# YaoZengzeng/yustack

Measured on AMD Instinct MI355X. Metric: GiB/s device-resident Internet checksum, batched packets, 1/2/4/8 MI355X, higher is better.
Workload: dtype u32; 1 GPU; config3: 1M x 1500-B TCP segments incl. pseudo-header (sendTCP field value); packets_per_gpu=1048576, packet_bytes=1500, mode=tcp, rotating_batches=2, kernel=k_small<16,6>, parallelism=shard1 (independent packets, no collective; one rank per GPU), backend=none

## Files before the change

### yustack_amd/csrc/yucsum_kernels.hip

```cpp
#include <hip/hip_runtime.h>

#include <stdint.h>

#include <atomic>
#include <type_traits>

#include "yucsum.h"
#include "yucsum_internal.h"
#include "yucsum_plan.h"

namespace {

constexpr uint32_t kSelSwap = 0x02030001u;
constexpr uint32_t kSelIdent = 0x03020100u;
using yu::kLEMax;

struct BatchArgs {
  const uint8_t *data;
  const uint64_t *offsets;
  const uint16_t *initial_arr;
  const uint8_t *addrs;
  uint16_t *out;
  uint8_t *fill;
  uint64_t stride;
  uint64_t n;
  uint64_t end;
  uint32_t len;
  uint32_t initial;
  uint32_t uf;
  uint32_t xcd;
  uint32_t small_waves;
  int mode;
};

__host__ __device__ __forceinline__ bool mode_is_ipv4(int m) {
  return m == YU_MODE_IPV4 || m == YU_MODE_VERIFY_IPV4;
}
using yu::l4_field;
using yu::l4_min;
using yu::mode_field;
using yu::mode_fills;
using yu::mode_is_tx;
__host__ __device__ __forceinline__ bool mode_has_pseudo(int m) {
  return m == YU_MODE_UDP || m == YU_MODE_TCP || m == YU_MODE_VERIFY_TCP ||
         m == YU_MODE_VERIFY_UDP;
}
__host__ __device__ __forceinline__ uint32_t mode_proto(int m) {
  return (m == YU_MODE_TCP || m == YU_MODE_VERIFY_TCP) ? 6u : 17u;
}
__host__ __device__ __forceinline__ uint32_t min_len(int m) {
  switch (m) {
    case YU_MODE_UDP: return 8;
    case YU_MODE_TCP: return 20;
    case YU_MODE_ICMP: return 4;
    case YU_MODE_IPV4:
    case YU_MODE_VERIFY_IPV4: return 1;
    default: return 0;
  }
}

__device__ __forceinline__ uint32_t fold32(uint32_t v) {
  uint32_t w = (v & 0xFFFFu) + (v >> 16);
  return (w + (w >> 16)) & 0xFFFFu;
}

__device__ __forceinline__ uint32_t sad(uint32_t x, uint32_t acc) {
  return __builtin_amdgcn_sad_u16(x, 0u, acc);
}

__device__ __forceinline__ uint32_t sadperm(uint32_t x, uint32_t sel,
                                            uint32_t acc) {
  return __builtin_amdgcn_sad_u16(__builtin_amdgcn_perm(x, x, sel), 0u, acc);
}

template <bool BE>
__device__ __forceinline__ uint32_t add_word(uint32_t x, uint32_t sel,
                                             uint32_t acc) {
  return BE ? sadperm(x, sel, acc) : sad(x, acc);
}

__device__ __forceinline__ uint32_t le_to_be(uint32_t s_le, uint32_t odd) {
  const uint32_t r = fold32(s_le);
  return odd ? r : (((r & 0xFFu) << 8) | (r >> 8));
}

template <int G>
__device__ __forceinline__ uint32_t group_total(uint32_t v) {
  static_assert(G >= 1 && G <= 64 && (G & (G - 1)) == 0, "G must be a power of two");
  if (G >= 2) v += (uint32_t)__builtin_amdgcn_update_dpp(0, (int)v, 0x111, 0xf, 0xf, true);
  if (G >= 4) v += (uint32_t)__builtin_amdgcn_update_dpp(0, (int)v, 0x112, 0xf, 0xf, true);
  if (G >= 8) v += (uint32_t)__builtin_amdgcn_update_dpp(0, (int)v, 0x114, 0xf, 0xf, true);
  if (G >= 16) v += (uint32_t)__builtin_amdgcn_update_dpp(0, (int)v, 0x118, 0xf, 0xf, true);
  if (G >= 32) v += (uint32_t)__builtin_amdgcn_update_dpp(0, (int)v, 0x142, 0xa, 0xf, false);
  if (G >= 64) v += (uint32_t)__builtin_amdgcn_update_dpp(0, (int)v, 0x143, 0xc, 0xf, false);
  return v;
}

__device__ __forceinline__ uint32_t wave_or(uint32_t v) {
  v |= (uint32_t)__builtin_amdgcn_update_dpp(0, (int)v, 0x111, 0xf, 0xf, true);
  v |= (uint32_t)__builtin_amdgcn_update_dpp(0, (int)v, 0x112, 0xf, 0xf, true);
  v |= (uint32_t)__builtin_amdgcn_update_dpp(0, (int)v, 0x114, 0xf, 0xf, true);
  v |= (uint32_t)__builtin_amdgcn_update_dpp(0, (int)v, 0x118, 0xf, 0xf, true);
  v |= (uint32_t)__builtin_amdgcn_update_dpp(0, (int)v, 0x142, 0xa, 0xf, false);
  v |= (uint32_t)__builtin_amdgcn_update_dpp(0, (int)v, 0x143, 0xc, 0xf, false);
  return (uint32_t)__shfl((int)v, 63, 64);
}

__device__ __forceinline__ uint64_t grid_wave(uint32_t xcd) {
  const uint32_t b = blockIdx.x, n = gridDim.x;
  uint32_t lb = b;
  if (xcd) {
    const uint32_t x = b & 7u, i = b >> 3, q = n >> 3, r = n & 7u;
    lb = (x < r ? x * (q + 1u) : r * (q + 1u) + (x - r) * q) + i;
  }
  return (uint64_t)lb * (blockDim.x >> 6) +
         (uint64_t)__builtin_amdgcn_readfirstlane(threadIdx.x >> 6);
}

typedef unsigned int u32x4 __attribute__((ext_vector_type(4)));

__device__ __forceinline__ uint64_t uniform64(uint64_t x) {
  const uint32_t lo = __builtin_amdgcn_readfirstlane((uint32_t)x);
  const uint32_t hi = __builtin_amdgcn_readfirstlane((uint32_t)(x >> 32));
  return ((uint64_t)hi << 32) | lo;
}

__device__ __forceinline__ uint64_t readlane64(uint64_t v, uint32_t l) {
  return ((uint64_t)(uint32_t)__builtin_amdgcn_readlane((int)(uint32_t)(v >> 32), l) << 32) |
         (uint32_t)__builtin_amdgcn_readlane((int)(uint32_t)v, l);
}

__device__ __forceinline__ uint64_t shfl64(uint64_t v, uint32_t src) {
  const uint32_t lo = (uint32_t)__shfl((int)(uint32_t)v, (int)src, 64);
  const uint32_t hi = (uint32_t)__shfl((int)(uint32_t)(v >> 32), (int)src, 64);
  return ((uint64_t)hi << 32) | lo;
}

using yu::kOOB;

__device__ __forceinline__ __amdgpu_buffer_rsrc_t rsrc_at(uint64_t base,
                                                          uint64_t end) {
  end = (end + 3u) & ~3ull;
  const uint64_t n = end > base ? end - base : 0;
  return __builtin_amdgcn_make_buffer_rsrc((void *)base, (short)0,
                                           (int)(n < kOOB ? n : kOOB), 0x00020000);
}

__device__ __forceinline__ uint4 bld16(__amdgpu_buffer_rsrc_t r, uint32_t off,
                                       bool nt) {
  const u32x4 t = nt ? __builtin_amdgcn_raw_buffer_load_b128(r, (int)off, 0, 2)
                     : __builtin_amdgcn_raw_buffer_load_b128(r, (int)off, 0, 0);
  return make_uint4(t.x, t.y, t.z, t.w);
}

template <int NT>
__device__ __forceinline__ constexpr bool nt_step(int u, int U) {
  return NT == 1 || (NT == 2 && u != 0 && u != U - 1);
}

struct Junk {
  uint32_t off[3];
  uint32_t mask[3];
};

__device__ __forceinline__ Junk make_junk(uint32_t sh, uint32_t E, int mode) {
  Junk j;
  j.off[0] = 0u;
  j.mask[0] = (1u << (8u * sh)) - 1u;
  const uint32_t f = mode_field(mode);
  const bool fld = mode_is_tx(mode) && sh + f + 2u <= E;
  const uint32_t fr = sh + f;
  const uint32_t fb = fr & 3u;
  j.off[1] = fr & ~3u;
  j.mask[1] = !fld ? 0u : (fb == 3u ? 0xFF000000u : (0xFFFFu << (8u * fb)));
  j.off[2] = (fr & ~3u) + 4u;
  j.mask[2] = (fld && fb == 3u) ? 0xFFu : 0u;
  return j;
}

__device__ __forceinline__ uint32_t pick_dword(const uint4 &c, uint32_t q) {
  return q == 0 ? c.x : (q == 1 ? c.y : (q == 2 ? c.z : c.w));
}

template <int LG>
__device__ __forceinline__ void junk_take(const uint4 &c0, uint32_t gbase,
                                          const Junk &j, uint32_t (&x)[3]) {
  static_assert(LG >= 1, "junk chunks 0/1 must sit in different lanes of step 0");
#pragma unroll
  for (int k = 0; k < 3; ++k) {
    const uint32_t d = j.off[k];
    x[k] = __shfl(pick_dword(c0, (d >> 2) & 3u), (int)(gbase + (d >> 4)), 64);
  }
}

template <bool BE>
__device__ __forceinline__ uint32_t junk_sum(const uint32_t (&x)[3],
                                             const Junk &j, uint32_t sel) {
  uint32_t s = 0;
#pragma unroll
  for (int k = 0; k < 3; ++k) s = add_word<BE>(x[k] & j.mask[k], sel, s);
  return s;
}

__device__ uint32_t g_side_zero[2] = {0u, 0u};

struct Side {
  uint32_t a, b;
  uint16_t i;
};

struct SidePtrs {
  const uint8_t *a;
  const uint8_t *i;
  uint32_t as, is;
};

__device__ __forceinline__ SidePtrs side_ptrs(const BatchArgs &A) {
  SidePtrs s;
  const bool use_addrs = A.addrs && mode_has_pseudo(A.mode);
  s.a = use_addrs ? A.addrs : (const uint8_t *)g_side_zero;
  s.as = use_addrs ? 8u : 0u;
  s.i = A.initial_arr ? (const uint8_t *)A.initial_arr : (const uint8_t *)g_side_zero;
  s.is = A.initial_arr ? 2u : 0u;
  return s;
}

__device__ __forceinline__ Side load_side(const SidePtrs &sp, uint64_t p) {
  const uint32_t *a = (const uint32_t *)(sp.a + p * sp.as);
  Side s;
  s.a = a[0];
  s.b = a[1];
  s.i = *(const uint16_t *)(sp.i + p * sp.is);
  return s;
}

__device__ __forceinline__ uint32_t packet_value(const BatchArgs &A, uint32_t v, uint64_t len,
                                                 const Side &sd) {
  const int mode = A.mode;
  if (mode == YU_MODE_RAW) {
    v += A.initial_arr ? sd.i : A.initial;
  } else if (mode_has_pseudo(mode)) {
    uint32_t ph;
    if (A.addrs) {
      ph = sadperm(sd.a, kSelSwap, 0u);
      ph = sadperm(sd.b, kSelSwap, ph);
      ph += mode_proto(mode);
    } else {
      ph = A.initial_arr ? sd.i : A.initial;
    }
    v += ph + (uint32_t)(len & 0xFFFFu);
  }
  uint32_t r = fold32(v);
  if (mode_is_tx(mode)) r = (~r) & 0xFFFFu;
  return r;
}

__device__ __forceinline__ void store_field(const BatchArgs &A, uint32_t r, uint8_t *pkt,
                                            uint32_t hdr_end) {
  const int mode = A.mode;
  if (A.fill && pkt && mode_is_tx(mode)) {
    const uint32_t f = mode_field(mode);
    if (f + 2u <= hdr_end) {
      uint8_t *q = pkt + f;
      const uint16_t be = (uint16_t)((r >> 8) | (r << 8));
      if (((uintptr_t)q & 1u) == 0 && !A.offsets) {
        __builtin_nontemporal_store(be, (uint16_t *)q);
      } else if (((uintptr_t)q & 1u) == 0) {
        *(uint16_t *)q = be;
      } else {
        q[0] = (uint8_t)(r >> 8);
        q[1] = (uint8_t)r;
      }
    }
  }
}

struct Extent {
  uint64_t hi;
};
__device__ __forceinline__ Extent batch_extent(const BatchArgs &A) {
  Extent e;
  e.hi = A.offsets ? A.offsets[A.n] : ~0ull;
  return e;
}

__device__ __forceinline__ uint8_t *fill_at(const BatchArgs &A, const Extent &x, uint64_t off,
                                            uint64_t len) {
  const bool in = len <= YU_MAX_TRANSPORT_LEN && off <= x.hi && len <= x.hi - off;
  return A.fill && in ? A.fill + off : nullptr;
}

__device__ __forceinline__ void finish_packet(const BatchArgs &A, uint64_t p,
                                              uint32_t v, uint64_t len,
                                              const Side &sd, uint8_t *pkt,
                                              uint32_t hdr_end) {
  const uint32_t r = packet_value(A, v, len, sd);
  if (A.out) A.out[p] = (uint16_t)r;
  store_field(A, r, pkt, hdr_end);
}

__device__ __forceinline__ uint32_t tail_cut(uint32_t x, int cr, int lim,
                                             uint32_t tm) {
  return cr < lim ? x : (cr == lim ? (x & tm) : 0u);
}

template <bool BE>
__device__ __forceinline__ uint32_t sum_masked(const uint4 &c, int cr,
                                               const int (&lim)[4], uint32_t tm,
                                               uint32_t sel, uint32_t acc) {
  acc = add_word<BE>(tail_cut(c.x, cr, lim[0], tm), sel, acc);
  acc = add_word<BE>(tail_cut(c.y, cr, lim[1], tm), sel, acc);
  acc = add_word<BE>(tail_cut(c.z, cr, lim[2], tm), sel, acc);
  acc = add_word<BE>(tail_cut(c.w, cr, lim[3], tm), sel, acc);
  return acc;
}

template <bool BE>
__device__ __forceinline__ uint32_t sum_full(const uint4 &c, uint32_t sel,
                                             uint32_t acc) {
  acc = add_word<BE>(c.x, sel, acc);
  acc = add_word<BE>(c.y, sel, acc);
  acc = add_word<BE>(c.z, sel, acc);
  acc = add_word<BE>(c.w, sel, acc);
  return acc;
}

__device__ __forceinline__ uint32_t ipv4_hl(uint32_t w0, uint32_t sh) {
  return ((w0 >> (8u * sh)) & 0xFu) * 4u;
}

template <int G, int U>
struct SmallItem {
  uint4 c[U];
  Side sd;
  uint32_t sh, len;
};

template <int G, int U, int NT, bool SIDE = true>
__device__ __forceinline__ void small_fetch(const BatchArgs &A,
                                            const SidePtrs &sp, uint64_t pb,
                                            uint32_t gw, uint32_t gl, bool ipv4,
                                            SmallItem<G, U> &it) {
  const uint64_t p = pb + gw;
  const bool active = p < A.n;
  const uint64_t data = (uint64_t)(uintptr_t)A.data;
  const uint64_t base = uniform64((data + pb * A.stride) & ~3ull);
  const uint64_t sabs = data + (active ? p : pb) * A.stride;
  const uint32_t lw = (uint32_t)((sabs & ~3ull) - base);
  it.sh = (uint32_t)(sabs & 3u);
  it.len = active ? A.len : 0u;
  const uint32_t le = ipv4 ? (it.len < 60u ? it.len : 60u) : it.len;
  const uint32_t eload = active ? it.sh + le : 0u;
  const __amdgpu_buffer_rsrc_t r = rsrc_at(base, A.end);
#pragma unroll
  for (int u = 0; u < U; ++u) {
    const uint32_t cr = 16u * (gl + (uint32_t)u * G);
    it.c[u] = bld16(r, cr < eload ? lw + cr : kOOB, nt_step<NT>(u, U));
  }
  if (SIDE) it.sd = load_side(sp, active ? p : A.n - 1);
}

template <int G, int U, int NT, int PR = 0>
__global__ __launch_bounds__(256) void k_small(BatchArgs A) {
  constexpr int GPW = 64 / G;
  constexpr int SPR = PR ? PR / GPW : 1;
  static_assert(PR == 0 || (PR % GPW == 0 && PR <= 64 && (SPR & (SPR - 1)) == 0),
                "a run is whole wave steps and fits the wave's lanes");
  const uint32_t lane = threadIdx.x & 63u;
  const uint32_t gl = lane & (G - 1);
  const uint32_t gw = lane / G;
  const uint64_t wave = grid_wave(A.xcd);
  const uint64_t nwaves = (uint64_t)gridDim.x * (blockDim.x >> 6);
  const int mode = A.mode;
  const bool ipv4 = mode_is_ipv4(mode);
  const SidePtrs sp = side_ptrs(A);
  const uint32_t uf = A.uf;
  auto first = [&](uint64_t t) -> uint64_t {
    if (PR == 0) return (wave + t * nwaves) * GPW;
    return (wave + t / SPR * nwaves) * PR + (t % SPR) * GPW;
  };

  uint64_t t = 0;
  uint64_t pb = first(0);
  if (pb >= A.n) return;
  uint32_t res = 0;
  Side rs, nrs;
  constexpr bool kDppSide = G <= 16;
  auto run_side = [&](uint64_t q, Side &d) __attribute__((always_inline)) {
    uint64_t x = q + lane;
    bool own = lane < (uint32_t)PR;
    if (kDppSide) {
      const uint32_t jj = (uint32_t)(G - 1) - gl;
      x = q + (uint64_t)jj * GPW + gw;
      own = jj < (uint32_t)SPR;
    }
    d = load_side(sp, own && x < A.n ? x : (q < A.n ? q : A.n - 1));
  };
  auto step = [&](const SmallItem<G, U> &it, SmallItem<G, U> &nx) __attribute__((always_inline)) -> bool {
    const uint64_t pn = first(t + 1);
    const bool more = pn < A.n;
    const uint32_t k = (uint32_t)(t % SPR);
    small_fetch<G, U, NT, PR == 0>(A, sp, more ? pn : A.n, gw, gl, ipv4, nx);
    if (PR && k == 0 && t) rs = nrs;
    if (PR && k == SPR - 1 && more) run_side(pn, nrs);

    uint32_t E = it.sh + it.len;
    if (ipv4) {
      const uint32_t hl = __shfl(ipv4_hl(it.c[0].x, it.sh), (int)(lane & ~(uint32_t)(G - 1)), 64);
      E = it.sh + (it.len < hl ? it.len : hl);
    }
    const int F = (int)(E & ~3u);
    const int lim[4] = {F, F - 4, F - 8, F - 12};
    const uint32_t tm = (1u << (8u * (E & 3u))) - 1u;
    uint32_t acc = 0;
#pragma unroll
    for (int u = 0; u < U; ++u) {
      const int cr = 16 * (int)(gl + (uint32_t)u * G);
      if ((uint32_t)u < uf)
        acc = sum_full<false>(it.c[u], 0u, acc);
      else
        acc = sum_masked<false>(it.c[u], cr, lim, tm, 0u, acc);
    }
    const uint64_t p = pb + gw;
    const Junk j = make_junk(it.sh, E, mode);
    uint32_t jx[3] = {0u, 0u, 0u};
    if (PR && kDppSide) {
      uint32_t own = 0;
#pragma unroll
      for (int i = 0; i < 3; ++i)
        if ((j.off[i] >> 4) == gl) own = sad(pick_dword(it.c[0], (j.off[i] >> 2) & 3u) & j.mask[i], own);
      acc -= own;
    } else {
      junk_take<__builtin_ctz(G)>(it.c[0], lane & ~(uint32_t)(G - 1), j, jx);
    }
    acc = group_total<G>(acc);
    if (PR == 0) {
      if (gl == G - 1 && p < A.n) {
        const uint32_t v = le_to_be(acc - junk_sum<false>(jx, j, 0u), it.sh & 1u);
        finish_packet(A, p, v, it.len, it.sd,
                      A.fill ? A.fill + p * A.stride : nullptr, E - it.sh);
      }
    } else {
      Side sd;
      if (kDppSide) {
        sd = rs;
        rs.a = (uint32_t)__builtin_amdgcn_update_dpp(0, (int)rs.a, 0x111, 0xf, 0xf, true);
        rs.b = (uint32_t)__builtin_amdgcn_update_dpp(0, (int)rs.b, 0x111, 0xf, 0xf, true);
        rs.i = (uint16_t)__builtin_amdgcn_update_dpp(0, (int)(uint32_t)rs.i, 0x111, 0xf, 0xf, true);
      } else {
        const int src = (int)(k * GPW + gw);
        sd.a = (uint32_t)__shfl((int)rs.a, src, 64);
        sd.b = (uint32_t)__shfl((int)rs.b, src, 64);
        sd.i = (uint16_t)__shfl((int)rs.i, src, 64);
      }
      const uint32_t v = le_to_be(acc - (kDppSide ? 0u : junk_sum<false>(jx, j, 0u)), it.sh & 1u);
      const uint32_t r = packet_value(A, v, it.len, sd);
      if (gl == G - 1 && p < A.n && A.fill) store_field(A, r, A.fill + p * A.stride, E - it.sh);
      const uint32_t got = (uint32_t)__shfl((int)r, (int)((lane % GPW) * G + G - 1), 64);
      res = lane / GPW == k ? got : res;
      if (k == SPR - 1 || !more) {
        const uint64_t q = pb - (uint64_t)k * GPW + lane;
        if (lane < (uint32_t)PR && q < A.n && A.out) A.out[q] = (uint16_t)res;
      }
    }
    pb = pn;
    ++t;
    return more;
  };
  SmallItem<G, U> a, b;
  small_fetch<G, U, NT, PR == 0>(A, sp, pb, gw, gl, ipv4, a);
  if (PR) run_side(pb, rs);
  for (;;) {
    if (!step(a, b)) break;
    if (!step(b, a)) break;
  }
}

template <int G>
struct TinyItem {
  uint4 c[G];
  Side sd;
};

template <int G, int NT>
__device__ __forceinline__ void tiny_fetch(const BatchArgs &A, const SidePtrs &sp,
                                           uint64_t pb, uint32_t g, uint32_t j,
                                           TinyItem<G> &it) {
  constexpr uint32_t GPW = 64 / G;
  const uint64_t base = uniform64((uint64_t)(uintptr_t)A.data + pb * A.stride);
  const __amdgpu_buffer_rsrc_t r = rsrc_at(base, A.end);
  const bool in = 16u * j < A.len;
#pragma unroll
  for (int k = 0; k < G; ++k) {
    const uint32_t q = GPW * (uint32_t)k + g;
    const bool active = in && pb + q < A.n;
    it.c[k] = bld16(r, active ? (uint32_t)(q * A.stride) + 16u * j : kOOB, NT != 0);
  }
  const uint64_t pf = pb + GPW * j + g;
  it.sd = load_side(sp, pf < A.n ? pf : A.n - 1);
}

template <int G>
__device__ __forceinline__ uint32_t bcast_last(uint32_t v, uint32_t lane) {
  if (G == 4)
    return (uint32_t)__builtin_amdgcn_update_dpp(0, (int)v, 0xFF, 0xf, 0xf, false);
  return (uint32_t)__shfl(v, (int)(lane | (G - 1)), 64);
}

template <int G>
__device__ __forceinline__ void tiny_store(const BatchArgs &A, uint64_t pb, uint32_t g, uint32_t j,
                                           const TinyItem<G> &it, uint32_t be, uint32_t f) {
  constexpr uint32_t GPW = 64 / G;
  const uint64_t e4 = A.end & ~3ull;
  const uint32_t fd = (f >> 2) & 3u, sh = (f & 2u) * 8u;
  const uint32_t m = 0xFFFFu << sh;
  const bool holder = j == (f >> 4);
  const bool in = 16u * j < A.len;
#pragma unroll
  for (int k = 0; k < G; ++k) {
    const uint32_t v = ((uint32_t)__shfl((int)be, (int)(g * G + (uint32_t)k), 64)) << sh;
    uint4 c = it.c[k];
    if (holder) {
      c.x = fd == 0 ? (c.x & ~m) | v : c.x;
      c.y = fd == 1 ? (c.y & ~m) | v : c.y;
      c.z = fd == 2 ? (c.z & ~m) | v : c.z;
      c.w = fd == 3 ? (c.w & ~m) | v : c.w;
    }
    const uint64_t q = pb + GPW * (uint32_t)k + g;
    uint32_t *dst = (uint32_t *)(A.fill + q * A.stride + 16u * j);
    const uint64_t da = (uint64_t)(uintptr_t)dst;
    if (in && q < A.n) {
      if (da + 16u <= e4) {
        *(uint4 *)dst = c;
      } else {
        if (da + 4u <= e4) dst[0] = c.x;
        if (da + 8u <= e4) dst[1] = c.y;
        if (da + 12u <= e4) dst[2] = c.z;
      }
    }
  }
}

template <int G, int NT, bool WB = false>
__global__ __launch_bounds__(256) void k_tiny(BatchArgs A) {
  constexpr uint32_t GPW = 64 / G;
  const uint32_t lane = threadIdx.x & 63u;
  const uint32_t j = lane & (G - 1);
  const uint32_t g = lane / G;
  const uint64_t wave = grid_wave(A.xcd);
  const uint64_t step = (uint64_t)gridDim.x * (blockDim.x >> 6) * 64u;
  const SidePtrs sp = side_ptrs(A);
  const uint32_t E = A.len;
  const int F = (int)(E & ~3u);
  const int lim[4] = {F, F - 4, F - 8, F - 12};
  const uint32_t tm = (1u << (8u * (E & 3u))) - 1u;
  const bool full = A.uf != 0;
  const uint32_t f = mode_field(A.mode);
  const uint32_t fm = (mode_is_tx(A.mode) && j == f / 16u) ? ~(0xFFFFu << (8u * (f & 3u))) : ~0u;
  const uint32_t fd = (f >> 2) & 3u;
  const uint4 m4 = make_uint4(fd == 0 ? fm : ~0u, fd == 1 ? fm : ~0u, fd == 2 ? fm : ~0u,
                              fd == 3 ? fm : ~0u);
  const bool wb = WB && A.fill && A.stride >= ((A.len + 15u) & ~15u);

  uint64_t pb = wave * 64u;
  if (pb >= A.n) return;
  TinyItem<G> it;
  tiny_fetch<G, NT>(A, sp, pb, g, j, it);
  for (;;) {
    const uint64_t pn = pb + step;
    const bool more = pn < A.n;
    TinyItem<G> nx;
    tiny_fetch<G, NT>(A, sp, more ? pn : A.n, g, j, nx);

    uint32_t mine = 0;
#pragma unroll
    for (int k = 0; k < G; ++k) {
      const uint4 c = make_uint4(it.c[k].x & m4.x, it.c[k].y & m4.y, it.c[k].z & m4.z,
                                 it.c[k].w & m4.w);
      uint32_t acc = full ? sum_full<false>(c, 0u, 0u)
                          : sum_masked<false>(c, 16 * (int)j, lim, tm, 0u, 0u);
      acc = bcast_last<G>(group_total<G>(acc), lane);
      mine = (j == (uint32_t)k) ? acc : mine;
    }
    const uint64_t pf = pb + GPW * j + g;
    if (wb) {
      const uint32_t r = packet_value(A, le_to_be(mine, 0u), E, it.sd);
      if (pf < A.n && A.out) A.out[pf] = (uint16_t)r;
      tiny_store<G>(A, pb, g, j, it, ((r >> 8) | (r << 8)) & 0xFFFFu, f);
    } else if (pf < A.n) {
      finish_packet(A, pf, le_to_be(mine, 0u), E, it.sd, A.fill ? A.fill + pf * A.stride : nullptr, E);
    }
    if (!more) break;
    it = nx;
    pb = pn;
  }
}

template <int U>
__device__ __forceinline__ void lane_fetch(const BatchArgs &A, const SidePtrs &sp,
                                           uint64_t pb, uint32_t lane, uint32_t span,
                                           bool nt, uint4 (&c)[U], Side &sd) {
  const uint64_t base = uniform64((uint64_t)(uintptr_t)A.data + pb * A.stride);
  const __amdgpu_buffer_rsrc_t r = rsrc_at(base, A.end);
#pragma unroll
  for (int u = 0; u < U; ++u) {
    const uint32_t off = 16u * (64u * (uint32_t)u + lane);
    c[u] = bld16(r, off < span ? off : kOOB, nt);
  }
  const uint64_t p = pb + lane;
  sd = load_side(sp, p < A.n ? p : A.n - 1);
}

template <int W>
__device__ __forceinline__ uint32_t lane_sum(const uint32_t *own, uint32_t nw, uint32_t k0) {
  uint32_t acc = 0, k = k0;
  for (uint32_t d = 0; d < nw; ++d) {
    if (W == 4) {
      const uint4 v = *(const uint4 *)(own + 4u * k);
      acc = sad(v.w, sad(v.z, sad(v.y, sad(v.x, acc))));
    } else if (W == 2) {
      const uint2 v = *(const uint2 *)(own + 2u * k);
      acc = sad(v.y, sad(v.x, acc));
    } else {
      acc = sad(own[k], acc);
    }
    k = k + 1u == nw ? 0u : k + 1u;
  }
  return acc;
}

template <int U>
__device__ __forceinline__ void lane_store(const BatchArgs &A, uint64_t pb, uint32_t lane,
                                           uint32_t span, const uint4 *slice) {
  const uint64_t base = uniform64((uint64_t)(uintptr_t)A.fill + pb * A.stride);
  const uint64_t lim = (A.end & ~3ull) > base ? (A.end & ~3ull) - base : 0u;
  const __amdgpu_buffer_rsrc_t r = __builtin_amdgcn_make_buffer_rsrc(
      (void *)base, (short)0, (int)(lim < span ? lim : span), 0x00020000);
#pragma unroll
  for (int u = 0; u < U; ++u) {
    const uint32_t off = 16u * (64u * (uint32_t)u + lane);
    const uint4 c = slice[64 * u + lane];
    __builtin_amdgcn_raw_buffer_store_b128(u32x4{c.x, c.y, c.z, c.w}, r, (int)(off < span ? off : kOOB), 0, 0);
  }
}

__device__ __forceinline__ void wave_lds_fence() {
  __builtin_amdgcn_fence(__ATOMIC_RELEASE, "wavefront");
  __builtin_amdgcn_wave_barrier();
  __builtin_amdgcn_fence(__ATOMIC_ACQUIRE, "wavefront");
}

template <int U, int NT>
__global__ __launch_bounds__(256) void k_lane(BatchArgs A) {
  __shared__ uint4 park[4][64 * U];
  const uint32_t lane = threadIdx.x & 63u;
  uint4 *slice = park[__builtin_amdgcn_readfirstlane(threadIdx.x >> 6)];
  const uint64_t wave = grid_wave(A.xcd);
  const uint64_t step = (uint64_t)gridDim.x * (blockDim.x >> 6) * 64u;
  const SidePtrs sp = side_ptrs(A);
  const uint32_t S = (uint32_t)A.stride;
  const uint32_t E = A.len;
  const uint32_t span = 64u * S;
  const uint32_t nd = (E + 3u) >> 2;
  const uint32_t junk_tail = (E & 3u) ? ~((1u << (8u * (E & 3u))) - 1u) : 0u;
  const uint32_t f = mode_field(A.mode);
  const bool tx = mode_is_tx(A.mode);
  const uint32_t junk_field = 0xFFFFu << (8u * (f & 3u));
  const uint32_t W = ((E | S) & 15u) == 0 ? 4u : (((E | S) & 7u) == 0 ? 2u : 1u);
  const uint32_t nw = nd / W;
  const uint32_t k0 = lane % nw;
  const uint32_t *own = (const uint32_t *)slice + lane * (S >> 2);

  uint64_t pb = wave * 64u;
  if (pb >= A.n) return;
  uint4 c[U];
  Side sd;
  lane_fetch<U>(A, sp, pb, lane, span, NT != 0, c, sd);
  for (;;) {
    const uint64_t pn = pb + step;
    const bool more = pn < A.n;
    uint4 nx[U];
    Side nsd;
    lane_fetch<U>(A, sp, more ? pn : A.n, lane, span, NT != 0, nx, nsd);

#pragma unroll
    for (int u = 0; u < U; ++u) slice[64 * u + lane] = c[u];
    wave_lds_fence();
    uint32_t acc = W == 4u ? lane_sum<4>(own, nw, k0)
                           : (W == 2u ? lane_sum<2>(own, nw, k0) : lane_sum<1>(own, nw, k0));
    if (junk_tail) acc -= sad(own[nd - 1u] & junk_tail, 0u);
    if (tx) acc -= sad(own[f >> 2] & junk_field, 0u);
    wave_lds_fence();

    const uint64_t p = pb + lane;
    if (A.fill) {
      const uint32_t r = packet_value(A, le_to_be(acc, 0u), E, sd);
      if (p < A.n && A.out) A.out[p] = (uint16_t)r;
      if (p < A.n && f + 2u <= E)
        ((uint16_t *)slice)[(lane * S + f) >> 1] = (uint16_t)((r >> 8) | (r << 8));
      wave_lds_fence();
      lane_store<U>(A, pb, lane, span, slice);
    } else if (p < A.n) {
      finish_packet(A, p, le_to_be(acc, 0u), E, sd, nullptr, E);
    }
    if (!more) break;
#pragma unroll
    for (int u = 0; u < U; ++u) c[u] = nx[u];
    sd = nsd;
    pb = pn;
  }
}

struct LoopPkt {
  uint64_t soff, len;
  uint64_t base;
  uint32_t sh, E, eload;
};

__device__ __forceinline__ void loop_pkt(const BatchArgs &A, uint64_t p,
                                         bool ipv4, LoopPkt &k) {
  if (p >= A.n) {
    k.soff = 0;
    k.len = 0;
    k.base = (uint64_t)(uintptr_t)A.data & ~3ull;
    k.sh = 0;
    k.E = 0;
    k.eload = 0;
    return;
  }
  if (A.offsets) {
    k.soff = A.offsets[p];
    k.len = A.offsets[p + 1] - k.soff;
  } else {
    k.soff = p * A.stride;
    k.len = A.len;
  }
  const uint64_t sabs = (uint64_t)(uintptr_t)A.data + k.soff;
  k.base = sabs & ~3ull;
  k.sh = (uint32_t)(sabs & 3u);
  const uint32_t l32 = k.len < YU_MAX_RAW_LEN ? (uint32_t)k.len : YU_MAX_RAW_LEN;
  k.E = k.sh + l32;
  k.eload = k.sh + (ipv4 ? (l32 < 60u ? l32 : 60u) : l32);
}

template <int U, int NT>
__device__ __forceinline__ void loop_fetch(const LoopPkt &k, uint32_t wb,
                                           uint32_t lane, uint64_t end,
                                           uint4 (&c)[U]) {
  const __amdgpu_buffer_rsrc_t r = rsrc_at(uniform64(k.base + wb), end);
  const uint32_t lim = k.eload > wb ? k.eload - wb : 0u;
#pragma unroll
  for (int u = 0; u < U; ++u) {
    const uint32_t cr = 16u * (lane + 64u * (uint32_t)u);
    c[u] = bld16(r, cr < lim ? cr : kOOB, NT != 0);
  }
}

template <int U, int NT, bool BE>
__global__ __launch_bounds__(256) void k_loop(BatchArgs A) {
  constexpr uint32_t W = 64u * 16u * U;
  const uint32_t lane = threadIdx.x & 63u;
  const uint64_t wave = grid_wave(A.xcd);
  const uint64_t nwave = (uint64_t)gridDim.x * (blockDim.x >> 6);
  const int mode = A.mode;
  const bool ipv4 = mode_is_ipv4(mode);
  const SidePtrs sp = side_ptrs(A);
  const bool lead = lane == 63;
  const uint64_t end = A.offsets ? (uint64_t)(uintptr_t)A.data + A.offsets[A.n] : A.end;
  const Extent ext = batch_extent(A);

  uint64_t p = wave;
  if (p >= A.n) return;
  LoopPkt cur, nxt;
  loop_pkt(A, p, ipv4, cur);
  Side sd = load_side(sp, p);
  uint32_t jx[3] = {0u, 0u, 0u};
  uint64_t pn = p + nwave;
  loop_pkt(A, pn, ipv4, nxt);

  uint32_t wb = 0;
  uint4 c[U];
  loop_fetch<U, NT>(cur, 0, lane, end, c);
  uint32_t acc = 0;
  for (;;) {
    const bool last = wb + W >= cur.eload;
    const bool more = !last || pn < A.n;
    uint4 cn[U];
    loop_fetch<U, NT>(last ? nxt : cur, last ? 0u : wb + W, lane, end, cn);
    const Side sdn = load_side(sp, (last && pn < A.n) ? pn : p);

    uint32_t E = cur.E;
    if (ipv4) {
      const uint32_t hl = __shfl(ipv4_hl(c[0].x, cur.sh), 0, 64);
      const uint32_t l32 = (uint32_t)cur.len;
      E = cur.sh + (l32 < hl ? l32 : hl);
    }
    const Junk j = make_junk(cur.sh, E, mode);
    if (wb == 0) junk_take<6>(c[0], 0u, j, jx);
    const uint32_t sel = (cur.sh & 1u) ? kSelIdent : kSelSwap;
    if (wb + W <= E) {
#pragma unroll
      for (int u = 0; u < U; ++u) acc = sum_full<BE>(c[u], sel, acc);
    } else {
      const int f = (int)((E & ~3u) - wb);
      const int lim[4] = {f, f - 4, f - 8, f - 12};
      const uint32_t tm = (1u << (8u * (E & 3u))) - 1u;
#pragma unroll
      for (int u = 0; u < U; ++u)
        acc = sum_masked<BE>(c[u], 16 * (int)(lane + 64u * (uint32_t)u), lim, tm, sel, acc);
    }

    if (last) {
      acc = group_total<64>(acc);
      if (lead) {
        const uint32_t s = acc - junk_sum<BE>(jx, j, sel);
        const uint32_t v = BE ? s : le_to_be(s, cur.sh & 1u);
        finish_packet(A, p, v, cur.len, sd, fill_at(A, ext, cur.soff, cur.len),
                      E - cur.sh);
      }
      if (!more) break;
      p = pn;
      cur = nxt;
      sd = sdn;
      pn = p + nwave;
      loop_pkt(A, pn, ipv4, nxt);
      wb = 0;
      acc = 0;
    } else {
      wb += W;
    }
#pragma unroll
    for (int u = 0; u < U; ++u) c[u] = cn[u];
  }
}

__device__ __forceinline__ uint32_t byte_range_mask(uint32_t lo, uint32_t a, uint32_t b) {
  const uint32_t ka = a > lo ? (a - lo < 4u ? a - lo : 4u) : 0u;
  const uint32_t kb = b > lo ? (b - lo < 4u ? b - lo : 4u) : 0u;
  const uint64_t hi = (1ull << (8u * kb)) - 1ull, low = (1ull << (8u * ka)) - 1ull;
  return (uint32_t)(hi & ~low);
}

template <int NT>
__global__ __launch_bounds__(256) void k_hdr(BatchArgs A) {
  constexpr bool TWO = true;
  const uint32_t lane = threadIdx.x & 63u;
  const uint64_t wave = grid_wave(A.xcd);
  const uint64_t nwave = (uint64_t)gridDim.x * (blockDim.x >> 6);
  const uint64_t data = (uint64_t)(uintptr_t)A.data;
  const bool tx = mode_is_tx(A.mode);
  const Extent ext = batch_extent(A);
  for (uint64_t p0 = wave * 64u; p0 < A.n; p0 += nwave * 64u) {
    const uint64_t p = p0 + lane;
    const bool act = p < A.n;
    uint64_t s, e;
    if (A.offsets) {
      s = A.offsets[act ? p : A.n];
      e = A.offsets[act ? p + 1 : A.n];
    } else {
      s = act ? p * A.stride : (A.n - 1) * A.stride + A.len;
      e = act ? s + A.len : s;
    }
    const uint64_t base = uniform64((data + s) & ~3ull);
    const uint64_t le = readlane64(e, 63);
    const uint64_t cend = data + (le < ext.hi ? le : ext.hi);
    const __amdgpu_buffer_rsrc_t r = rsrc_at(base, cend);
    const uint64_t sa = data + s;
    const uint32_t sh = (uint32_t)sa & 3u;
    const uint64_t len = e - s;
    const bool step_ok = !__any((int)(len > YU_MAX_TRANSPORT_LEN));
    const uint32_t lmax = sh + (uint32_t)(len < 60u ? len : 60u);
    const uint64_t wo = (sa & ~3ull) - base;
    uint4 c[4];
#pragma unroll
    for (int k = 0; k < (TWO ? 2 : 4); ++k)
      c[k] = bld16(r, (16u * k < lmax && wo < kOOB) ? (uint32_t)wo + 16u * k : kOOB, NT != 0);
    const uint32_t hl = ipv4_hl(c[0].x, sh);
    if (TWO) {
      const uint32_t need = sh + (uint32_t)(len < hl ? len : hl);
#pragma unroll
      for (int k = 2; k < 4; ++k)
        c[k] = __any((int)(need > 32u))
                   ? bld16(r, (16u * k < need && wo < kOOB) ? (uint32_t)wo + 16u * k : kOOB, NT != 0)
                   : make_uint4(0u, 0u, 0u, 0u);
    }
    const uint32_t E = sh + (uint32_t)(len < hl ? len : hl);
    const bool fld = tx && sh + 12u <= E;
    const uint32_t f0 = fld ? sh + 10u : 0u, f1 = fld ? sh + 12u : 0u;
    uint32_t acc = 0;
#pragma unroll
    for (int k = 0; k < 4; ++k) {
      const uint32_t w[4] = {c[k].x, c[k].y, c[k].z, c[k].w};
#pragma unroll
      for (int j = 0; j < 4; ++j) {
        const uint32_t lo = 16u * k + 4u * j;
        const uint32_t m = byte_range_mask(lo, sh, E) & ~byte_range_mask(lo, f0, f1);
        acc = sad(w[j] & m, acc);
      }
    }
    if (act) {
      const uint32_t v = le_to_be(acc, (uint32_t)sa & 1u);
      Side sd;
      sd.a = sd.b = 0u;
      sd.i = 0;
      finish_packet(A, p, v, len, sd, step_ok ? fill_at(A, ext, s, len) : nullptr, E - sh);
    }
  }
}

constexpr uint32_t kInv255 = 0xFEFEFEFFu;

struct SegChunk {
  uint64_t ox, oy;
  uint64_t b0;
  uint64_t xe;
  Side sd;
};

template <int CH, bool SIDE = true>
__device__ __forceinline__ void seg_load(const BatchArgs &A, const SidePtrs &sp,
                                         uint64_t p0, uint32_t lane, SegChunk &k) {
  const uint64_t n = A.n;
  const uint64_t i = p0 + lane;
  const uint64_t ce = p0 < n ? (n - p0 < (uint64_t)CH ? n : p0 + CH) : n;
  const bool own = lane < (uint32_t)CH && i < n;
  const uint64_t last = p0 < n ? ce - 1u : 0u;
  const uint64_t uy = (own ? i : last) * A.stride + A.len;
  const uint64_t *offs = A.offsets ? A.offsets : (const uint64_t *)g_side_zero;
  const uint64_t ry = offs[A.offsets ? (own ? i + 1 : ce) : 0];
  const uint64_t rx = offs[A.offsets ? (own ? i : ce) : 0];
  k.ox = A.offsets ? rx : (own ? i * A.stride : uy);
  k.oy = A.offsets ? ry : uy;
  if (SIDE) k.sd = load_side(sp, own ? i : n - 1);
}


__device__ __forceinline__ void seg_geom(uint64_t data, uint64_t n, uint64_t p0, SegChunk &k,
                                         uint32_t, bool ragged, uint32_t lim, bool each, uint32_t ch,
                                         uint64_t end, bool line128 = false) {
  if (p0 >= n) {
    k.b0 = data & ~3ull;
    k.xe = 0;
    return;
  }
  const uint64_t s = data + readlane64(k.ox, 0);
  const uint64_t e = data + readlane64(k.oy, 63);
  const uint64_t l = s & ~127ull;
  k.b0 = line128 && l >= (data & ~3ull) ? l : s & ~3ull;
  k.xe = e - k.b0;
  if (ragged && (each ? (__any((int)(k.oy - k.ox > (uint64_t)lim)) != 0 || e > end)
                      : k.xe > (uint64_t)ch * lim + 131u))
    k.xe = 0;
// ... 890 lines not shown
```

Measured before the change: 6314 GiB/s.

## Load packet batches as dense cache-line-aligned wave slices and repack via LDS

For the k_small<16,6> instance with uniform, contiguous, 4-byte-multiple packets and no fill or IPv4, each wave now loads the whole contiguous span of its four packets with coalesced 16-byte loads aligned to 128-byte lines. It then redistributes the bytes through a per-wave LDS slice so each 16-lane group sees its own packet laid out as before. The aim is to replace per-packet misaligned, partially wasted loads (1500 B is not a multiple of 16) with fully coalesced line-aligned traffic. The cost is extra LDS writes and reads, two wave fences per step, and LDS pressure; a waves-per-eu attribute of 5 is also added to that instance.

```diff
diff --git a/yustack_amd/csrc/yucsum_dense.h b/yustack_amd/csrc/yucsum_dense.h
--- /dev/null
+++ b/yustack_amd/csrc/yucsum_dense.h
@@ -0,0 +1,73 @@
+#ifndef YUCSUM_DENSE_H
+#define YUCSUM_DENSE_H
+
+#include <stdint.h>
+
+#if defined(__HIPCC__) || defined(__CUDACC__)
+#define YU_DENSE_FN __host__ __device__ __forceinline__
+#else
+#define YU_DENSE_FN inline
+#endif
+
+#pragma GCC visibility push(hidden)
+namespace yu {
+
+constexpr uint32_t kDenseLine = 128u;
+constexpr uint32_t kDensePiece = 1024u;
+constexpr uint32_t kDenseOOB = 0x80000000u;
+
+constexpr bool dense_inst(int G, int U) { return G == 16 && U == 6; }
+
+YU_DENSE_FN bool dense_ok(int G, int U, uint64_t data, bool ragged, uint64_t stride, uint32_t len,
+                          bool fill, bool ipv4) {
+  return dense_inst(G, U) && !ragged && stride == len && !fill && !ipv4 && (data & 15u) == 0 &&
+         len != 0 && (len & 3u) == 0 &&
+         (uint64_t)(64 / G) * len + (kDenseLine - 4u) <= (uint64_t)kDensePiece * (uint32_t)U;
+}
+
+struct DenseStep {
+  uint64_t base;
+  uint32_t lead;
+  uint32_t lo;
+  uint32_t hi;
+};
+
+YU_DENSE_FN DenseStep dense_step(uint64_t data, uint32_t len, uint64_t n, uint64_t pb,
+                                 uint32_t gpw) {
+  DenseStep s;
+  const uint64_t start = data + pb * len;
+  s.base = start & ~(uint64_t)(kDenseLine - 1u);
+  s.lead = (uint32_t)(start - s.base);
+  s.lo = data > s.base ? (uint32_t)(data - s.base) : 0u;
+  s.hi = 0u;
+  if (pb < n) {
+    const uint64_t rem = n - pb;
+    const uint32_t bytes = s.lead + (uint32_t)(rem < gpw ? rem : gpw) * len;
+    s.hi = rem > gpw ? (bytes + kDenseLine - 1u) & ~(kDenseLine - 1u) : bytes;
+  }
+  return s;
+}
+
+YU_DENSE_FN uint32_t dense_x0(const DenseStep &s, uint32_t lane) { return 16u * lane - s.lo; }
+YU_DENSE_FN uint32_t dense_lim(const DenseStep &s) { return s.hi > s.lo ? s.hi - s.lo : 0u; }
+
+YU_DENSE_FN uint32_t dense_chunk(const DenseStep &s, uint32_t u, uint32_t lane) {
+  const uint32_t x = dense_x0(s, lane) + u * kDensePiece;
+  return x < dense_lim(s) ? s.lo + x : kDenseOOB;
+}
+
+YU_DENSE_FN uint32_t dense_window(uint64_t data, uint32_t len, uint64_t pb, uint32_t gw) {
+  return (((uint32_t)data + (uint32_t)pb * len) & (kDenseLine - 1u)) + gw * len;
+}
+
+constexpr uint32_t dense_pad(int G, int U) {
+  const uint32_t gpw = 64u / (uint32_t)G, slice = kDensePiece * (uint32_t)U;
+  const uint32_t lmax = ((slice - (kDenseLine - 4u)) / gpw) & ~3u;
+  const uint32_t reach = (kDenseLine - 4u) + (gpw - 1u) * lmax + 16u * (uint32_t)G * (uint32_t)U;
+  return reach > slice ? (reach - slice + 15u) & ~15u : 0u;
+}
+
+}
+#pragma GCC visibility pop
+
+#endif
diff --git a/yustack_amd/csrc/yucsum_kernels.hip b/yustack_amd/csrc/yucsum_kernels.hip
--- a/yustack_amd/csrc/yucsum_kernels.hip
+++ b/yustack_amd/csrc/yucsum_kernels.hip
@@ -6,6 +6,7 @@
 #include <type_traits>
 
 #include "yucsum.h"
+#include "yucsum_dense.h"
 #include "yucsum_internal.h"
 #include "yucsum_plan.h"
 
@@ -329,6 +330,12 @@
   return ((w0 >> (8u * sh)) & 0xFu) * 4u;
 }
 
+__device__ __forceinline__ void wave_lds_fence() {
+  __builtin_amdgcn_fence(__ATOMIC_RELEASE, "wavefront");
+  __builtin_amdgcn_wave_barrier();
+  __builtin_amdgcn_fence(__ATOMIC_ACQUIRE, "wavefront");
+}
+
 template <int G, int U>
 struct SmallItem {
   uint4 c[U];
@@ -340,28 +347,62 @@
 __device__ __forceinline__ void small_fetch(const BatchArgs &A,
                                             const SidePtrs &sp, uint64_t pb,
                                             uint32_t gw, uint32_t gl, bool ipv4,
-                                            SmallItem<G, U> &it) {
+                                            bool dense, SmallItem<G, U> &it) {
   const uint64_t p = pb + gw;
   const bool active = p < A.n;
   const uint64_t data = (uint64_t)(uintptr_t)A.data;
-  const uint64_t base = uniform64((data + pb * A.stride) & ~3ull);
+  const uint64_t wbase = (data + pb * A.stride) & ~3ull;
   const uint64_t sabs = data + (active ? p : pb) * A.stride;
-  const uint32_t lw = (uint32_t)((sabs & ~3ull) - base);
   it.sh = (uint32_t)(sabs & 3u);
   it.len = active ? A.len : 0u;
   const uint32_t le = ipv4 ? (it.len < 60u ? it.len : 60u) : it.len;
-  const uint32_t eload = active ? it.sh + le : 0u;
-  const __amdgpu_buffer_rsrc_t r = rsrc_at(base, A.end);
+  uint64_t b = wbase;
+  uint32_t x0 = 16u * gl, dx = 16u * G;
+  uint32_t lim = active ? it.sh + le : 0u;
+  uint32_t add = (uint32_t)((sabs & ~3ull) - wbase);
+  if (yu::dense_inst(G, U) && dense) {
+    const yu::DenseStep ds = yu::dense_step(data, A.len, A.n, pb, 64 / G);
+    b = ds.base;
+    x0 = yu::dense_x0(ds, gw * G + gl);
+    dx = yu::kDensePiece;
+    lim = yu::dense_lim(ds);
+    add = ds.lo;
+  }
+  const __amdgpu_buffer_rsrc_t r = rsrc_at(uniform64(b), A.end);
 #pragma unroll
   for (int u = 0; u < U; ++u) {
-    const uint32_t cr = 16u * (gl + (uint32_t)u * G);
-    it.c[u] = bld16(r, cr < eload ? lw + cr : kOOB, nt_step<NT>(u, U));
+    const uint32_t x = x0 + (uint32_t)u * dx;
+    it.c[u] = bld16(r, x < lim ? add + x : kOOB, nt_step<NT>(u, U));
   }
   if (SIDE) it.sd = load_side(sp, active ? p : A.n - 1);
 }
 
+template <int G, int U, int W>
+__device__ __forceinline__ void small_repack(SmallItem<G, U> &it, uint4 *slice, uint32_t wo,
+                                             uint32_t lane, uint32_t gl) {
+#pragma unroll
+  for (int u = 0; u < U; ++u) slice[64 * u + lane] = it.c[u];
+  wave_lds_fence();
+  const uint8_t *win = (const uint8_t *)slice + wo + 16u * gl;
+#pragma unroll
+  for (int u = 0; u < U; ++u) {
+    const uint8_t *q = win + 16 * G * u;
+    if (W == 4) {
+      it.c[u] = *(const uint4 *)q;
+    } else if (W == 2) {
+      const uint2 a = *(const uint2 *)q, b = *(const uint2 *)(q + 8);
+      it.c[u] = make_uint4(a.x, a.y, b.x, b.y);
+    } else {
+      const uint32_t *d = (const uint32_t *)q;
+      it.c[u] = make_uint4(d[0], d[1], d[2], d[3]);
+    }
+  }
+  wave_lds_fence();
+}
+
 template <int G, int U, int NT, int PR = 0>
-__global__ __launch_bounds__(256) void k_small(BatchArgs A) {
+__global__ __launch_bounds__(256)
+    __attribute__((amdgpu_waves_per_eu(yu::dense_inst(G, U) ? 5 : 1))) void k_small(BatchArgs A) {
   constexpr int GPW = 64 / G;
   constexpr int SPR = PR ? PR / GPW : 1;
   static_assert(PR == 0 || (PR % GPW == 0 && PR <= 64 && (SPR & (SPR - 1)) == 0),
@@ -375,6 +416,14 @@
   const bool ipv4 = mode_is_ipv4(mode);
   const SidePtrs sp = side_ptrs(A);
   const uint32_t uf = A.uf;
+  constexpr bool kDense = yu::dense_inst(G, U);
+  uint4 *slice = nullptr;
+  if constexpr (kDense) {
+    __shared__ uint4 park[4 * 64 * U + yu::dense_pad(G, U) / 16];
+    slice = park + 64 * U * __builtin_amdgcn_readfirstlane(threadIdx.x >> 6);
+  }
+  const bool dense = kDense && yu::dense_ok(G, U, (uint64_t)(uintptr_t)A.data, A.offsets != nullptr,
+                                            A.stride, A.len, A.fill != nullptr, ipv4);
   auto first = [&](uint64_t t) -> uint64_t {
     if (PR == 0) return (wave + t * nwaves) * GPW;
     return (wave + t / SPR * nwaves) * PR + (t % SPR) * GPW;
@@ -396,13 +445,20 @@
     }
     d = load_side(sp, own && x < A.n ? x : (q < A.n ? q : A.n - 1));
   };
-  auto step = [&](const SmallItem<G, U> &it, SmallItem<G, U> &nx) __attribute__((always_inline)) -> bool {
+  auto step = [&](SmallItem<G, U> &it, SmallItem<G, U> &nx) __attribute__((always_inline)) -> bool {
     const uint64_t pn = first(t + 1);
     const bool more = pn < A.n;
     const uint32_t k = (uint32_t)(t % SPR);
-    small_fetch<G, U, NT, PR == 0>(A, sp, more ? pn : A.n, gw, gl, ipv4, nx);
+    const uint64_t p = pb + gw;
+    small_fetch<G, U, NT, PR == 0>(A, sp, more ? pn : A.n, gw, gl, ipv4, dense, nx);
     if (PR && k == 0 && t) rs = nrs;
     if (PR && k == SPR - 1 && more) run_side(pn, nrs);
+    if (kDense && dense) {
+      const uint32_t wo = p < A.n ? yu::dense_window((uint64_t)(uintptr_t)A.data, A.len, pb, gw) : 0u;
+      if ((A.len & 15u) == 0) small_repack<G, U, 4>(it, slice, wo, lane, gl);
+      else if ((A.len & 7u) == 0) small_repack<G, U, 2>(it, slice, wo, lane, gl);
+      else small_repack<G, U, 1>(it, slice, wo, lane, gl);
+    }
 
     uint32_t E = it.sh + it.len;
     if (ipv4) {
@@ -421,7 +477,6 @@
       else
         acc = sum_masked<false>(it.c[u], cr, lim, tm, 0u, acc);
     }
-    const uint64_t p = pb + gw;
     const Junk j = make_junk(it.sh, E, mode);
     uint32_t jx[3] = {0u, 0u, 0u};
     if (PR && kDppSide) {
@@ -468,7 +523,7 @@
     return more;
   };
   SmallItem<G, U> a, b;
-  small_fetch<G, U, NT, PR == 0>(A, sp, pb, gw, gl, ipv4, a);
+  small_fetch<G, U, NT, PR == 0>(A, sp, pb, gw, gl, ipv4, dense, a);
   if (PR) run_side(pb, rs);
   for (;;) {
     if (!step(a, b)) break;
@@ -642,12 +697,6 @@
     const uint4 c = slice[64 * u + lane];
     __builtin_amdgcn_raw_buffer_store_b128(u32x4{c.x, c.y, c.z, c.w}, r, (int)(off < span ? off : kOOB), 0, 0);
   }
-}
-
-__device__ __forceinline__ void wave_lds_fence() {
-  __builtin_amdgcn_fence(__ATOMIC_RELEASE, "wavefront");
-  __builtin_amdgcn_wave_barrier();
-  __builtin_amdgcn_fence(__ATOMIC_ACQUIRE, "wavefront");
 }
 
 template <int U, int NT>
```

After: 6446 GiB/s (median of 6 runs). 2.1% higher.
